# microsoft/tutel

Measured on NVIDIA H100. Metric: moe_layer_fwd_bwd_tokens_per_sec, higher is better.
Workload: dtype bf16; 1 GPU; model=helloworld moe_layer top-2 8-expert ffn(relu) model_dim=4096 hidden=14336, global_batch=16, seq_len=512, parallelism=ep1 (8 local experts/GPU), a2a_ffn_overlap_degree=1, cuda_graph=True, launches_per_graph_replay=15

## Files before the change

### csrc/gemm_sm90.cu

```cuda
#include "gemm_sm90.h"

#include <cuda.h>
#include <cuda_bf16.h>
#include <cuda_fp16.h>

#include <cstdio>
#include <cstdlib>
#include <mutex>

#include "ptx.cuh"

namespace tb {

struct GemmArgs {
  int M, N, K, G;
  int b_group_div;
  int tiles_m, tiles_n;
  long long num_tiles;

  void* d;
  long long ldd, d_group_stride;
  const unsigned long long* d_ptr_table;
  int out_dtype;

// ... 17 lines not shown
  long long colsum_group_stride;
  const float* scale_a;
  long long scale_a_group_stride;
  const float* scale_b;
  long long scale_b_group_stride;

  const uint32_t* wait_flags;
  int wait_rows_per_flag, wait_flags_per_group;
  uint32_t wait_target;
  const unsigned long long* signal_ptr_table;
  int group_rot, group_mod;
};

namespace {

constexpr int kThreads = 384;
constexpr int kSwizzleBytes = 128;
constexpr int kSmemLimit = 232448;

template <int BN_>
struct Cfg {
  static constexpr int BM = 128;
  static constexpr int BN = BN_;
  static constexpr bool WIDE = BN_ == 256;
  static constexpr int A_BYTES = BM * kSwizzleBytes;
  static constexpr int B_BYTES = BN * kSwizzleBytes;
  static constexpr int STAGE_BYTES = A_BYTES + B_BYTES;
  static constexpr int EPI_COLS = 128;
  static constexpr int EPI_PITCH = EPI_COLS + 8;
  static constexpr int EPI_WARP_BYTES = 16 * EPI_PITCH * 4;
  static constexpr int EPI_BYTES = WIDE ? 0 : 8 * EPI_WARP_BYTES;
  static constexpr int OUT_BOX_BYTES = BM * kSwizzleBytes;
  static constexpr int OUT_TILE_BYTES = WIDE ? BM * BN * 2 : 0;
  static constexpr int COLSUM_BYTES = WIDE ? 2 * BN * 4 : 0;
  static constexpr int BAR_BYTES = 512;
  static constexpr int STAGES = WIDE ? 3 : 4;
  static constexpr int MAXNREG = WIDE ? 168 : 144;
  static constexpr int CONSUMER_REGS = WIDE ? 232 : 192;
  static constexpr int SMEM_BYTES = STAGES * STAGE_BYTES + 1024 + OUT_TILE_BYTES + BAR_BYTES + EPI_BYTES + COLSUM_BYTES;
  static_assert((STAGES * STAGE_BYTES) % 1024 == 0, "the output tile must stay 1024B aligned for the 128B swizzle");
  static_assert(WIDE || SMEM_BYTES + 2 * 1024 <= 228 * 1024, "no room for the push kernel");
  static_assert(SMEM_BYTES <= kSmemLimit, "");
  static_assert(128 * 40 + 256 * CONSUMER_REGS <= 65536 && 384 * MAXNREG <= 65536, "register budget");
};

struct TileCoord {
  int g, m_blk, n_blk;
};

template <int kBand>
__device__ __forceinline__ TileCoord decode_tile(long long t, int tiles_m, int tiles_n) {
  const int per_group = tiles_m * tiles_n;
  TileCoord c;
  c.g = static_cast<int>(t / per_group);
  int r = static_cast<int>(t - static_cast<long long>(c.g) * per_group);
  const int band_tiles = kBand * tiles_n;
  const int band = r / band_tiles;
  const int first_m = band * kBand;
  const int rows_in_band = min(kBand, tiles_m - first_m);
  r -= band * band_tiles;
  c.m_blk = first_m + r % rows_in_band;
  c.n_blk = r / rows_in_band;
  return c;
}

__device__ __forceinline__ int rotate_group(int g, int rot, int mod) {
  if (mod > 1) {
    const int base = (g / mod) * mod;
    return base + (g - base + rot) % mod;
  }
  if (mod < -1) {
    const int m = -mod;
// ... 88 lines not shown
    else a = g[j] * fast_sigmoid(g[j]);
    o[j] = a * u[j];
  }
}
template <int ACT>
__device__ __forceinline__ void glu_bwd_seg(const float* r, const float* g, float* u, float* o) {
#pragma unroll
  for (int j = 0; j < 32; ++j) {
    const float dh = r[j];
    float a, da;
    if constexpr (ACT == ACT_RELU) {
      a = fmaxf(g[j], 0.0f);
      da = g[j] > 0.0f ? 1.0f : 0.0f;
    } else if constexpr (ACT == ACT_GELU) {
      const float cdf = 0.5f * (1.0f + erff(g[j] * 0.70710678118654752f));
      a = g[j] * cdf;
      da = cdf + g[j] * 0.3989422804014327f * __expf(-0.5f * g[j] * g[j]);
    } else {
      const float sg = fast_sigmoid(g[j]);
      a = g[j] * sg;
      da = sg * (1.0f + g[j] * (1.0f - sg));
    }
    o[j] = dh * u[j] * da;
    u[j] = dh * a;
  }
}

enum WideMain : int { WM_NONE, WM_BIAS, WM_RELU_BWD, WM_ADD, WM_GELU_BWD, WM_SILU_BWD };

__device__ __forceinline__ uint32_t out_tile_off(int j, int swz) {
  return static_cast<uint32_t>((j >> 3) * (128 * kSwizzleBytes) + (((j & 7) ^ swz) << 4));
}

__device__ __forceinline__ void wide_scale(float (&acc)[128], float sa0, float sa1, const float* sb, int n_lane, int N) {
#pragma unroll
  for (int j = 0; j < 32; ++j) {
    const int n = n_lane + 8 * j;
    if (sb != nullptr && n < N) {
      const float2 s = *reinterpret_cast<const float2*>(sb + n);
      acc[4 * j] *= sa0 * s.x; acc[4 * j + 1] *= sa0 * s.y;
      acc[4 * j + 2] *= sa1 * s.x; acc[4 * j + 3] *= sa1 * s.y;
    } else {
      acc[4 * j] *= sa0; acc[4 * j + 1] *= sa0;
      acc[4 * j + 2] *= sa1; acc[4 * j + 3] *= sa1;
    }
  }
}

template <int WM>
__device__ __forceinline__ void wide_main(float (&acc)[128], const uint8_t* row0, int swz, const uint8_t* bias_g,
                                          bool bias_f32, bool bias_bf16, int n_lane, int N, bool out_bf16, float alpha) {
#pragma unroll
  for (int j = 0; j < 32; ++j) {
    if constexpr (WM == WM_NONE) {
#pragma unroll
      for (int c = 0; c < 4; ++c) acc[4 * j + c] *= alpha;
    } else if constexpr (WM == WM_BIAS) {
      const int n = n_lane + 8 * j;
      float2 b = make_float2(0.0f, 0.0f);
      if (n < N)
        b = bias_f32 ? *reinterpret_cast<const float2*>(bias_g + n * 4)
                     : unpack2(*reinterpret_cast<const uint32_t*>(bias_g + n * 2), bias_bf16);
      acc[4 * j] += b.x; acc[4 * j + 1] += b.y;
      acc[4 * j + 2] += b.x; acc[4 * j + 3] += b.y;
    } else {
      const uint32_t o = out_tile_off(j, swz);
#pragma unroll
      for (int h = 0; h < 2; ++h) {
        const float2 f = unpack2(*reinterpret_cast<const uint32_t*>(row0 + h * 8 * kSwizzleBytes + o), out_bf16);
        float& v0 = acc[4 * j + 2 * h];
        float& v1 = acc[4 * j + 2 * h + 1];
        if constexpr (WM == WM_RELU_BWD) { v0 = relu_bwd(v0, f.x); v1 = relu_bwd(v1, f.y); }
        else if constexpr (WM == WM_ADD) { v0 += f.x; v1 += f.y; }
        else if constexpr (WM == WM_GELU_BWD) { v0 = gelu_bwd(v0, f.x); v1 = gelu_bwd(v1, f.y); }
        else { v0 = silu_bwd(v0, f.x); v1 = silu_bwd(v1, f.y); }
      }
    }
  }
}

template <int ACT>
__device__ __forceinline__ void wide_act(float (&acc)[128]) {
#pragma unroll
  for (int i = 0; i < 128; ++i) {
    if constexpr (ACT == ACT_RELU) acc[i] = fmaxf(acc[i], 0.0f);
    else if constexpr (ACT == ACT_GELU) acc[i] = gelu_erf(acc[i]);
    else acc[i] = silu(acc[i]);
  }
}

__device__ __forceinline__ void wide_stage(const float (&acc)[128], uint8_t* row0, int swz, bool out_bf16) {
#pragma unroll
  for (int j = 0; j < 32; ++j) {
    const uint32_t o = out_tile_off(j, swz);
    *reinterpret_cast<uint32_t*>(row0 + o) = pack2(acc[4 * j], acc[4 * j + 1], out_bf16);
    *reinterpret_cast<uint32_t*>(row0 + 8 * kSwizzleBytes + o) = pack2(acc[4 * j + 2], acc[4 * j + 3], out_bf16);
  }
}

__device__ __forceinline__ void wide_colsum(const float (&acc)[128], bool ok0, bool ok1, int lane, float* colrow) {
  float s[64];
#pragma unroll
  for (int j = 0; j < 32; ++j) {
#pragma unroll
    for (int c = 0; c < 2; ++c) s[2 * j + c] = (ok0 ? acc[4 * j + c] : 0.0f) + (ok1 ? acc[4 * j + 2 + c] : 0.0f);
  }
#pragma unroll
  for (int off = 16; off >= 4; off >>= 1) {
    const bool upper = (lane & off) != 0;
#pragma unroll
    for (int i = 0; i < 2 * off; ++i) {
      const float send = upper ? s[i] : s[i + 2 * off];
      const float recv = __shfl_xor_sync(0xffffffffu, send, off);
      s[i] = (upper ? s[i + 2 * off] : s[i]) + recv;
    }
  }
  float* base = colrow + 32 * (lane >> 2) + 2 * (lane & 3);
#pragma unroll
  for (int i = 0; i < 8; ++i) atomicAdd(base + 8 * (i >> 1) + (i & 1), s[i]);
}

struct OutTileStore {
  const uint8_t* tile;
  uint32_t tile_smem;
  int m0, n0, m_valid, N, g;
  long long group_stride, ld;
  bool straddle;
  int ct;
  bool writer;
};
__device__ __forceinline__ void flush_out_tile(const OutTileStore& s, const CUtensorMap* map, uint8_t* dst, bool wait_read) {
  constexpr int kChunks = 256 / 8;
  ptx::fence_proxy_async_smem();
  ptx::named_bar_sync(1, 256);
  if (s.straddle) {
    for (int i = s.ct; i < 128 * kChunks; i += 256) {
      const int r = i / kChunks, ch = i % kChunks;
      const int m = s.m0 + r, n = s.n0 + ch * 8;
      if (m < s.m_valid && n < s.N) {
        const uint4 v = *reinterpret_cast<const uint4*>(s.tile + (ch >> 3) * (128 * kSwizzleBytes) + r * kSwizzleBytes +
                                                        (((ch & 7) ^ (r & 7)) << 4));
        *reinterpret_cast<uint4*>(dst + (static_cast<long long>(s.g) * s.group_stride + static_cast<long long>(m) * s.ld + n) * 2) = v;
      }
    }
    ptx::named_bar_sync(1, 256);
    return;
  }
  if (s.writer) {
    for (int b = 0; b < 4; ++b)
      if (s.n0 + 64 * b < s.N) ptx::tma_store_3d(map, s.tile_smem + b * (128 * kSwizzleBytes), s.n0 + 64 * b, s.m0, s.g);
    ptx::bulk_commit_group();
    if (wait_read) ptx::bulk_wait_group_read<0>();
  }
  if (wait_read) ptx::named_bar_sync(1, 256);
}

template <int BN_, bool A_MN, bool B_MN, int DT>
__global__ void __maxnreg__(Cfg<BN_>::MAXNREG)
gemm_sm90_kernel(const __grid_constant__ CUtensorMap tmA, const __grid_constant__ CUtensorMap tmB,
                 const __grid_constant__ CUtensorMap tmB2, const __grid_constant__ CUtensorMap tmD,
                 const __grid_constant__ CUtensorMap tmAux, const __grid_constant__ CUtensorMap tmD2,
                 const GemmArgs args) {
  using C = Cfg<BN_>;
  constexpr int BN = C::BN;
  extern __shared__ uint8_t smem_raw[];

  const int warp = __shfl_sync(0xffffffffu, static_cast<int>(threadIdx.x >> 5), 0);
  const int lane = threadIdx.x & 31;

  const uint32_t smem_base = (ptx::smem_u32(smem_raw) + 1023u) & ~1023u;
  constexpr int stages = C::STAGES;
  const uint32_t out_base = smem_base + static_cast<uint32_t>(stages) * C::STAGE_BYTES;
  const uint32_t bar_base = out_base + C::OUT_TILE_BYTES;
  auto smem_a = [&](int s) { return smem_base + s * C::STAGE_BYTES; };
  auto smem_b = [&](int s) { return smem_base + s * C::STAGE_BYTES + C::A_BYTES; };
  auto full_bar = [&](int s) { return bar_base + 8u * s; };
  auto empty_bar = [&](int s) { return bar_base + 64u + 8u * s; };
  const uint32_t aux_full = bar_base + 128u;
  const uint32_t out_empty = bar_base + 136u;
  const uint32_t epi_base = bar_base + C::BAR_BYTES;
  float* epi_ptr = reinterpret_cast<float*>(smem_raw + (epi_base - ptx::smem_u32(smem_raw)));
  uint8_t* out_tile = smem_raw + (out_base - ptx::smem_u32(smem_raw));
  float* colsum_rows = epi_ptr;
  const bool aux_tma = C::WIDE && (args.epilogue == EPI_RELU_BWD || args.epilogue == EPI_ADD || args.epilogue == EPI_ACT_BWD);

  if (warp == 0 && ptx::elect_one()) {
    ptx::prefetch_tensormap(&tmA);
    ptx::prefetch_tensormap(&tmB);
    if (args.dual) ptx::prefetch_tensormap(&tmB2);
    if (C::WIDE) ptx::prefetch_tensormap(&tmD);
    if (aux_tma) ptx::prefetch_tensormap(&tmAux);
  }
  if (warp == 1 && lane == 0) {
    for (int s = 0; s < stages; ++s) {
      ptx::mbar_init(full_bar(s), 1);
      ptx::mbar_init(empty_bar(s), 2);
    }
    ptx::mbar_init(aux_full, 1);
    ptx::mbar_init(out_empty, 1);
    ptx::fence_mbar_init();
  }
  if constexpr (C::WIDE) {
    for (int i = threadIdx.x; i < 2 * BN; i += kThreads) colsum_rows[i] = 0.0f;
  }
  __syncthreads();

  constexpr int kEltBytes = (DT == DT_E4M3 || DT == DT_E5M2) ? 1 : 2;
  static_assert(kEltBytes == 2 || (!A_MN && !B_MN), "8-bit operands are K-major only");
  const int num_kb = (args.K * kEltBytes + kSwizzleBytes - 1) / kSwizzleBytes;
  constexpr int bk_elems = kSwizzleBytes / kEltBytes;
  const long long tile_step = gridDim.x;
  const long long tile_first = blockIdx.x;
  constexpr int kBand = 16;
  const bool dual = !C::WIDE && args.dual != 0;
  const int tile_n = dual ? BN / 2 : BN;
  const int kb_out_free = min(2, num_kb - 1);

  if (warp < 4) {
    ptx::setmaxnreg_dec<40>();
    if (warp == 0) {
      int s = 0;
      uint32_t ph = 0;
      uint32_t it = 0;
      int seen_group = -1;
      unsigned long long seen_mask = 0ull;
      for (long long t = tile_first; t < args.num_tiles; t += tile_step) {
        TileCoord tc = decode_tile<kBand>(t, args.tiles_m, args.tiles_n);
        tc.g = rotate_group(tc.g, args.group_rot, args.group_mod);
        if (args.row_counts != nullptr && tc.m_blk * C::BM >= args.row_counts[tc.g]) continue;
        const int m0 = tc.m_blk * C::BM;
        const int n0 = tc.n_blk * BN;
        const int gb = tc.g / args.b_group_div;
        if (args.wait_flags != nullptr) {
          if (tc.g != seen_group) { seen_group = tc.g; seen_mask = 0ull; }
          const int f0 = (tc.m_blk * C::BM) / args.wait_rows_per_flag;
          const int f1 = (min(tc.m_blk * C::BM + C::BM, args.M) - 1) / args.wait_rows_per_flag;
          unsigned long long need = 0ull;
          for (int f = f0; f <= f1; ++f) need |= 1ull << (f & 63);
          if ((seen_mask & need) != need) {
            if (lane == 0) {
              for (int f = f0; f <= f1; ++f)
                if (!((seen_mask >> (f & 63)) & 1ull))
                  ptx::wait_flag_ge_sys_quiet(args.wait_flags + static_cast<long long>(tc.g) * args.wait_flags_per_group + f,
                                        args.wait_target);
              ptx::fence_proxy_async_global();
            }
            __syncwarp();
            seen_mask |= need;
          }
        }
        for (int kb = 0; kb < num_kb; ++kb) {
          ptx::mbar_wait_quiet(empty_bar(s), ph ^ 1u);
          if (ptx::elect_one()) {
            const uint32_t fb = full_bar(s);
            ptx::mbar_expect_tx(fb, C::STAGE_BYTES);
            const int k0 = kb * bk_elems;
            constexpr int chunk_elems = kSwizzleBytes / kEltBytes;
            constexpr int chunk_bytes = bk_elems * kSwizzleBytes;
            if constexpr (!A_MN) {
              ptx::tma_load_3d(smem_a(s), &tmA, fb, k0, m0, tc.g);
            } else {
              for (int c = 0; c < C::BM / chunk_elems; ++c)
                ptx::tma_load_3d(smem_a(s) + c * chunk_bytes, &tmA, fb, m0 + c * chunk_elems, k0, tc.g);
            }
            if (!dual) {
              if constexpr (!B_MN) {
                ptx::tma_load_3d(smem_b(s), &tmB, fb, k0, n0, gb);
              } else {
                for (int c = 0; c < BN / chunk_elems; ++c)
                  ptx::tma_load_3d(smem_b(s) + c * chunk_bytes, &tmB, fb, n0 + c * chunk_elems, k0, gb);
              }
            } else {
              const int nb0 = tc.n_blk * (BN / 2);
              if constexpr (!B_MN) {
                ptx::tma_load_3d(smem_b(s), &tmB, fb, k0, nb0, gb);
                ptx::tma_load_3d(smem_b(s) + (BN / 2) * kSwizzleBytes, &tmB2, fb, k0, nb0, gb);
              } else {
                constexpr int half_chunks = (BN / 2) / chunk_elems;
                for (int c = 0; c < 2 * half_chunks; ++c)
                  ptx::tma_load_3d(smem_b(s) + c * chunk_bytes, c < half_chunks ? &tmB : &tmB2, fb,
                                   nb0 + (c % half_chunks) * chunk_elems, k0, gb);
              }
            }
          }
          __syncwarp();
          if (++s == stages) { s = 0; ph ^= 1u; }
          if (aux_tma && kb == kb_out_free) {
            ptx::mbar_wait_quiet(out_empty, (it & 1u) ^ 1u);
            if (ptx::elect_one()) {
              ptx::mbar_expect_tx(aux_full, C::OUT_TILE_BYTES);
              for (int b = 0; b < BN / 64; ++b)
                ptx::tma_load_3d(out_base + b * C::OUT_BOX_BYTES, &tmAux, aux_full, n0 + 64 * b, m0, tc.g);
            }
            __syncwarp();
          }
        }
        ++it;
      }
    }
  } else {
    ptx::setmaxnreg_inc<C::CONSUMER_REGS>();
    const int cw = warp - 4;
    const int wg = cw >> 2;
    const bool wg_leader = (threadIdx.x & 127) == 0;
    int s = 0;
    uint32_t ph = 0;
    constexpr uint32_t kMnChunkBytes = 64u * kSwizzleBytes;
    constexpr uint32_t kMnKStep = 16u * kSwizzleBytes;
    constexpr uint32_t a_lbo = A_MN ? kMnChunkBytes : 16u;
    constexpr uint32_t b_lbo = B_MN ? kMnChunkBytes : 16u;
    constexpr uint32_t a_kstep = (A_MN ? kMnKStep : 32u) >> 4;
    constexpr uint32_t b_kstep = (B_MN ? kMnKStep : 32u) >> 4;
    constexpr uint32_t desc_hi = (1024u >> 4) | (1u << 30);
    const uint32_t a_lo0 = (((smem_a(0) + static_cast<uint32_t>(wg) * 8192u) >> 4) & 0x3FFFu) | ((a_lbo >> 4) << 16);
    const uint32_t b_lo0 = ((smem_b(0) >> 4) & 0x3FFFu) | ((b_lbo >> 4) << 16);

    const bool out16 = (args.out_dtype != DT_FP32);
    const bool out_bf16 = (args.out_dtype == DT_BF16);
    const bool glu = !C::WIDE && (args.epilogue == EPI_GLU || args.epilogue == EPI_GLU_BWD);
    float* epi_warp = epi_ptr + cw * 16 * C::EPI_PITCH;
    const float* epi_row = epi_warp + (lane & 15) * C::EPI_PITCH;
    const int col_half = (lane >> 4) * 32;
    auto load_acc = [&](int col, float* v) {
#pragma unroll
      for (int q = 0; q < 8; ++q) {
        const float4 t4 = *reinterpret_cast<const float4*>(epi_row + col + q * 4);
        v[q * 4] = t4.x; v[q * 4 + 1] = t4.y; v[q * 4 + 2] = t4.z; v[q * 4 + 3] = t4.w;
      }
    };
    const int ct = threadIdx.x - 128;
    const bool out_writer = ct == 0;
    const int r0 = cw * 16 + (lane >> 2);
    const int swz = lane >> 2;
    uint8_t* row0 = out_tile + r0 * kSwizzleBytes + (lane & 3) * 4;
    const int wmain = args.epilogue == EPI_NONE ? WM_NONE
                    : args.epilogue == EPI_ADD ? WM_ADD
                    : args.epilogue == EPI_RELU_BWD ? WM_RELU_BWD
                    : args.epilogue == EPI_ACT_BWD ? (args.act == ACT_GELU ? WM_GELU_BWD : args.act == ACT_SILU ? WM_SILU_BWD : WM_RELU_BWD)
                    : WM_BIAS;
    uint32_t it = 0;

    for (long long t = tile_first; t < args.num_tiles; t += tile_step) {
      TileCoord tc = decode_tile<kBand>(t, args.tiles_m, args.tiles_n);
      tc.g = rotate_group(tc.g, args.group_rot, args.group_mod);
      int m_valid = args.M;
      if (args.row_counts != nullptr) {
        m_valid = min(args.M, args.row_counts[tc.g]);
        if (tc.m_blk * C::BM >= m_valid) continue;
      }
      float acc[BN / 2];
      if constexpr (C::WIDE) {
#pragma unroll
        for (int i = 0; i < BN / 2; ++i) acc[i] = 0.0f;
      }
      int prev_s = 0;
      for (int kb = 0; kb < num_kb; ++kb) {
        ptx::mbar_wait_quiet(full_bar(s), ph);
        const uint32_t a_lo = a_lo0 + static_cast<uint32_t>(s) * (C::STAGE_BYTES >> 4);
        const uint32_t b_lo = b_lo0 + static_cast<uint32_t>(s) * (C::STAGE_BYTES >> 4);
        ptx::wgmma_fence();
#pragma unroll
        for (int k = 0; k < 4; ++k) {
          const uint64_t ad = (static_cast<uint64_t>(desc_hi) << 32) | (a_lo + k * a_kstep);
          const uint64_t bd = (static_cast<uint64_t>(desc_hi) << 32) | (b_lo + k * b_kstep);
          if constexpr (BN == 256) ptx::wgmma_m64n256<DT, A_MN, B_MN>(acc, ad, bd, (kb | k) != 0);
          else ptx::wgmma_m64n128<DT, A_MN, B_MN>(acc, ad, bd, (kb | k) != 0);
        }
        ptx::wgmma_commit();
        if constexpr (C::WIDE) {
          if (out_writer && it > 0 && kb == kb_out_free) {
            ptx::bulk_wait_group_read<0>();
            ptx::mbar_arrive(out_empty);
          }
          __syncwarp();
        }
        if (kb > 0) {
          ptx::wgmma_wait<1>();
          if (wg_leader) ptx::mbar_arrive(empty_bar(prev_s));
        }
        prev_s = s;
        if (++s == stages) { s = 0; ph ^= 1u; }
      }
      ptx::wgmma_wait<0>();
      if (wg_leader) ptx::mbar_arrive(empty_bar(prev_s));

      if constexpr (C::WIDE) {
        const int m0 = tc.m_blk * C::BM, n0 = tc.n_blk * BN;
        const int gb = tc.g / args.b_group_div;
        const bool ok0 = m0 + r0 < m_valid, ok1 = m0 + r0 + 8 < m_valid;
        const int n_lane = n0 + 2 * (lane & 3);
        const bool straddle = m0 + C::BM > m_valid && m_valid < args.M;
        if (args.scale_a != nullptr || args.scale_b != nullptr) {
          const float* sa = args.scale_a != nullptr ? args.scale_a + static_cast<long long>(tc.g) * args.scale_a_group_stride + m0 + r0 : nullptr;
          const float sa0 = (sa != nullptr && ok0) ? sa[0] : 1.0f;
          const float sa1 = (sa != nullptr && ok1) ? sa[8] : 1.0f;
          const float* sb = args.scale_b != nullptr ? args.scale_b + static_cast<long long>(gb) * args.scale_b_group_stride : nullptr;
          wide_scale(acc, sa0, sa1, sb, n_lane, args.N);
        }
        const uint8_t* bias_g = nullptr;
        if (args.bias != nullptr)
          bias_g = reinterpret_cast<const uint8_t*>(args.bias) +
                   static_cast<long long>(gb) * args.bias_group_stride * (args.bias_is_fp32 ? 4 : 2);
        const uint32_t out_free_parity = (it & 1u) ^ 1u;

        const OutTileStore st{out_tile, out_base, m0, n0, m_valid, args.N, tc.g, args.d_group_stride, args.ldd, straddle, ct,
                              out_writer};

        if (wmain == WM_BIAS) {
          if (bias_g != nullptr)
            wide_main<WM_BIAS>(acc, row0, swz, bias_g, args.bias_is_fp32 != 0, args.bias_is_bf16 != 0, n_lane, args.N, out_bf16, 1.0f);
          if (args.d2 != nullptr && (args.epilogue == EPI_BIAS_GELU || args.epilogue == EPI_BIAS_SILU)) {
            ptx::mbar_wait_quiet(out_empty, out_free_parity);
            wide_stage(acc, row0, swz, out_bf16);
            flush_out_tile(st, &tmD2, reinterpret_cast<uint8_t*>(args.d2), true);
          }
          if (args.epilogue == EPI_BIAS_RELU) wide_act<ACT_RELU>(acc);
          else if (args.epilogue == EPI_BIAS_GELU) wide_act<ACT_GELU>(acc);
          else if (args.epilogue == EPI_BIAS_SILU) wide_act<ACT_SILU>(acc);
        } else if (wmain == WM_NONE) {
          if (args.alpha != 1.0f) wide_main<WM_NONE>(acc, row0, swz, nullptr, false, false, n_lane, args.N, out_bf16, args.alpha);
        } else {
          ptx::mbar_wait_quiet(aux_full, it & 1u);
          if (wmain == WM_RELU_BWD) wide_main<WM_RELU_BWD>(acc, row0, swz, nullptr, false, false, n_lane, args.N, out_bf16, 1.0f);
          else if (wmain == WM_ADD) wide_main<WM_ADD>(acc, row0, swz, nullptr, false, false, n_lane, args.N, out_bf16, 1.0f);
          else if (wmain == WM_GELU_BWD) wide_main<WM_GELU_BWD>(acc, row0, swz, nullptr, false, false, n_lane, args.N, out_bf16, 1.0f);
          else wide_main<WM_SILU_BWD>(acc, row0, swz, nullptr, false, false, n_lane, args.N, out_bf16, 1.0f);
        }
        if (!aux_tma) ptx::mbar_wait_quiet(out_empty, out_free_parity);
        wide_stage(acc, row0, swz, out_bf16);
        float* colrow = colsum_rows + (it & 1u) * BN;
        if (args.colsum != nullptr) wide_colsum(acc, ok0, ok1, lane, colrow);
        flush_out_tile(st, &tmD, reinterpret_cast<uint8_t*>(args.d), false);
        if (args.colsum != nullptr && ct < BN / 4) {
          float4* src = reinterpret_cast<float4*>(colrow) + ct;
          const float4 v = *src;
          *src = make_float4(0.0f, 0.0f, 0.0f, 0.0f);
          const int n = n0 + 4 * ct;
          if (n < args.N) {
            float* cs = args.colsum + static_cast<long long>(gb) * args.colsum_group_stride + n;
            if ((reinterpret_cast<uintptr_t>(cs) & 15) == 0) {
              ptx::red_add_v4_f32(cs, v.x, v.y, v.z, v.w);
            } else {
              atomicAdd(cs, v.x); atomicAdd(cs + 1, v.y); atomicAdd(cs + 2, v.z); atomicAdd(cs + 3, v.w);
            }
          }
        }
        ++it;
        continue;
      }

      {
        const int fr = lane >> 2, fc = (lane & 3) * 2;
#pragma unroll
        for (int j = 0; j < C::EPI_COLS / 8; ++j) {
          *reinterpret_cast<float2*>(epi_warp + fr * C::EPI_PITCH + j * 8 + fc) = make_float2(acc[4 * j], acc[4 * j + 1]);
          *reinterpret_cast<float2*>(epi_warp + (fr + 8) * C::EPI_PITCH + j * 8 + fc) = make_float2(acc[4 * j + 2], acc[4 * j + 3]);
        }
      }
      __syncwarp();

      const int m = tc.m_blk * C::BM + cw * 16 + (lane & 15);
      const bool row_ok = m < m_valid;
      const int gb = tc.g / args.b_group_div;
      uint8_t* d_base = (args.d_ptr_table != nullptr)
                            ? reinterpret_cast<uint8_t*>(args.d_ptr_table[tc.g])
                            : reinterpret_cast<uint8_t*>(args.d) +
                                  static_cast<long long>(tc.g) * args.d_group_stride * (out16 ? 2 : 4);
      uint8_t* d_row = d_base + static_cast<long long>(m) * args.ldd * (out16 ? 2 : 4);
      const uint8_t* aux_row = nullptr;
      if (args.aux != nullptr)
        aux_row = reinterpret_cast<const uint8_t*>(args.aux) +
                  (static_cast<long long>(tc.g) * args.aux_group_stride + static_cast<long long>(m) * args.ld_aux) * 2;
      const uint8_t* aux2_row = nullptr;
      if (args.aux2 != nullptr)
        aux2_row = reinterpret_cast<const uint8_t*>(args.aux2) +
                   (static_cast<long long>(tc.g) * args.aux_group_stride + static_cast<long long>(m) * args.ld_aux) * 2;
      const uint8_t* bias_g = nullptr;
      if (args.bias != nullptr)
        bias_g = reinterpret_cast<const uint8_t*>(args.bias) +
// ... 157 lines not shown
        if (args.colsum != nullptr) {
          float s[32];
#pragma unroll
          for (int j = 0; j < 32; ++j) s[j] = row_ok ? v[j] : 0.0f;
#pragma unroll
          for (int off = 8; off >= 1; off >>= 1) {
            const bool upper = (lane & off) != 0;
#pragma unroll
            for (int i = 0; i < 2 * off; ++i) {
              const float send = upper ? s[i] : s[i + 2 * off];
              const float recv = __shfl_xor_sync(0xffffffffu, send, off);
              s[i] = (upper ? s[i + 2 * off] : s[i]) + recv;
            }
          }
          const int cc = 2 * (lane & 15);
          float* cs = args.colsum + static_cast<long long>(gb) * args.colsum_group_stride + n + cc;
          if (cc < ncols) {
            atomicAdd(cs, s[0]);
            atomicAdd(cs + 1, s[1]);
          }
        }
        store_seg(d_row, n, ncols, v);
      }
      }
      __syncwarp();
      if (args.signal_ptr_table != nullptr) {
        asm volatile("bar.sync 1, 256;" ::: "memory");
        if (cw == 0 && lane == 0) {
          ptx::fence_acq_rel_sys();
          ptx::red_add_release_sys(reinterpret_cast<uint32_t*>(args.signal_ptr_table[tc.g]), 1u);
        }
      }
    }
    if constexpr (C::WIDE) {
      if (out_writer) ptx::bulk_wait_group<0>();
    }
  }
}

using EncodeTiledFn = CUresult (*)(CUtensorMap*, CUtensorMapDataType, cuuint32_t, void*, const cuuint64_t*,
                                   const cuuint64_t*, const cuuint32_t*, const cuuint32_t*, CUtensorMapInterleave,
                                   CUtensorMapSwizzle, CUtensorMapL2promotion, CUtensorMapFloatOOBfill);

EncodeTiledFn get_encode_fn() {
  static EncodeTiledFn fn = nullptr;
  static std::once_flag once;
  std::call_once(once, [] {
    void* p = nullptr;
    cudaDriverEntryPointQueryResult q;
    if (cudaGetDriverEntryPoint("cuTensorMapEncodeTiled", &p, cudaEnableDefault, &q) == cudaSuccess &&
        q == cudaDriverEntryPointSuccess)
      fn = reinterpret_cast<EncodeTiledFn>(p);
  });
  return fn;
}

bool make_operand_map(CUtensorMap* map, const void* base, int dtype, bool mn_major, long long rows_mn,
                      long long k, long long ld, long long group_stride, int groups, int box_mn_kmajor,
                      const char** why) {
  EncodeTiledFn enc = get_encode_fn();
  if (enc == nullptr) { *why = "cuTensorMapEncodeTiled unavailable"; return false; }
  const int eb = (dtype == DT_E4M3 || dtype == DT_E5M2) ? 1 : 2;
  CUtensorMapDataType dt = eb == 1 ? CU_TENSOR_MAP_DATA_TYPE_UINT8
                                   : (dtype == DT_BF16 ? CU_TENSOR_MAP_DATA_TYPE_BFLOAT16 : CU_TENSOR_MAP_DATA_TYPE_FLOAT16);
  if ((reinterpret_cast<uintptr_t>(base) & 15) || ((ld * eb) & 15) || ((group_stride * eb) & 15)) {
    *why = "operand base/stride must be 16-byte aligned";
    return false;
  }
  cuuint64_t dims[3];
// ... 77 lines not shown
  int sms = sm_count_cache[dev & 63];
  if (p.max_ctas > 0) sms = p.max_ctas < sms ? p.max_ctas : sms;

  const bool dual = p.epilogue == EPI_GLU;
  if (dual && (p.b2 == nullptr || p.out_dtype == DT_FP32)) { *why = "EPI_GLU needs b2 and a 16-bit output"; return cudaErrorInvalidValue; }
  if (p.epilogue == EPI_GLU_BWD && (p.aux == nullptr || p.aux2 == nullptr || p.d2 == nullptr || p.out_dtype == DT_FP32)) {
    *why = "EPI_GLU_BWD needs aux, aux2, d2 and a 16-bit output";
    return cudaErrorInvalidValue;
  }
  if ((p.epilogue == EPI_GLU || p.epilogue == EPI_GLU_BWD) && p.d_ptr_table != nullptr) { *why = "GLU epilogues write local outputs only"; return cudaErrorInvalidValue; }
  const bool uses_aux = p.epilogue == EPI_RELU_BWD || p.epilogue == EPI_ADD || p.epilogue == EPI_GLU_BWD || p.epilogue == EPI_ACT_BWD;
  if (uses_aux && (p.aux == nullptr || p.out_dtype == DT_FP32 ||
                   ((reinterpret_cast<uintptr_t>(p.aux) | reinterpret_cast<uintptr_t>(p.aux2)) & 15) || ((p.ld_aux * 2) & 15) ||
                   ((p.aux_group_stride * 2) & 15))) {
    *why = "this epilogue needs a 16-byte aligned 16-bit aux operand";
    return cudaErrorInvalidValue;
  }
  const int groups_b = (p.G + (p.b_group_div > 0 ? p.b_group_div : 1) - 1) / (p.b_group_div > 0 ? p.b_group_div : 1);
  if ((p.G > 1 && (p.a_group_stride == 0 || (p.d_ptr_table == nullptr && p.d_group_stride == 0) ||
                   (uses_aux && p.aux_group_stride == 0))) ||
      (groups_b > 1 && p.b_group_stride == 0)) {
    *why = "group strides of A, B, aux and the output must be nonzero when there is more than one group";
    return cudaErrorInvalidValue;
  }
  const int mod_abs = p.group_mod < 0 ? -p.group_mod : p.group_mod;
  if (mod_abs > 1 && (p.G % mod_abs != 0 || p.group_rot < 0)) {
    *why = "G must be a multiple of |group_mod|, and group_rot must not be negative";
    return cudaErrorInvalidValue;
  }
  if (p.alpha != 1.0f && p.epilogue != EPI_NONE) { *why = "alpha is applied by EPI_NONE only"; return cudaErrorInvalidValue; }
  if (p.cta_group < 0 || p.cta_group > 2) { *why = "cta_group must be 0, 1 or 2"; return cudaErrorInvalidValue; }
  if (p.block_n != 0 && p.block_n != 128 && p.block_n != 256) { *why = "block_n must be 0, 128 or 256"; return cudaErrorInvalidValue; }

  const bool wide = p.block_n != 128 && p.wait_flags == nullptr && p.signal_ptr_table == nullptr && p.d_ptr_table == nullptr &&
                    p.epilogue != EPI_GLU && p.epilogue != EPI_GLU_BWD && p.out_dtype != DT_FP32;
  constexpr int bm = 128;
  const int bn = wide ? 256 : 128;
  GemmArgs a{};
  a.M = p.M; a.N = p.N; a.K = p.K; a.G = p.G;
  a.b_group_div = p.b_group_div > 0 ? p.b_group_div : 1;
  a.tiles_m = (p.M + bm - 1) / bm;
  a.tiles_n = dual ? (p.N + bn / 2 - 1) / (bn / 2) : (p.N + bn - 1) / bn;
  a.num_tiles = static_cast<long long>(a.tiles_m) * a.tiles_n * p.G;
  a.d = p.d; a.ldd = p.ldd; a.d_group_stride = p.d_group_stride; a.d_ptr_table = p.d_ptr_table;
  a.out_dtype = p.out_dtype;
  a.epilogue = p.epilogue; a.alpha = p.alpha;
  a.bias = p.bias; a.bias_group_stride = p.bias_group_stride; a.bias_is_fp32 = 0;
  a.bias_is_bf16 = (eb == 2) ? (p.in_dtype == DT_BF16) : (p.out_dtype == DT_BF16);
  a.aux = p.aux; a.ld_aux = p.ld_aux; a.aux_group_stride = p.aux_group_stride;
  a.aux2 = p.aux2; a.d2 = p.d2; a.d3 = p.d3; a.dual = dual ? 1 : 0; a.act = p.act; a.scale_b2 = p.scale_b2;
  a.row_counts = p.row_counts;
  a.colsum = p.colsum; a.colsum_group_stride = p.colsum_group_stride;
  a.scale_a = p.scale_a; a.scale_a_group_stride = p.scale_a_group_stride;
  a.scale_b = p.scale_b; a.scale_b_group_stride = p.scale_b_group_stride;
  a.wait_flags = p.wait_flags; a.wait_rows_per_flag = p.wait_rows_per_flag > 0 ? p.wait_rows_per_flag : bm;
  a.wait_flags_per_group = p.wait_flags_per_group; a.wait_target = p.wait_target;
  a.signal_ptr_table = p.signal_ptr_table;
  a.group_rot = p.group_rot; a.group_mod = p.group_mod;

  CUtensorMap ta, tb_;
  const int gB = (p.G + a.b_group_div - 1) / a.b_group_div;
  if (!make_operand_map(&ta, p.a, p.in_dtype, p.a_mn_major, p.M, p.K, p.lda, p.a_group_stride, p.G, bm, why))
    return cudaErrorInvalidValue;
  const int b_box = dual ? bn / 2 : bn;
  if (!make_operand_map(&tb_, p.b, p.in_dtype, p.b_mn_major, p.N, p.K, p.ldb, p.b_group_stride, gB, b_box, why))
    return cudaErrorInvalidValue;
  CUtensorMap tb2 = tb_;
  if (dual && !make_operand_map(&tb2, p.b2, p.in_dtype, p.b_mn_major, p.N, p.K, p.ldb, p.b_group_stride, gB, b_box, why))
// ... 45 lines not shown
```

### csrc/ptx.cuh

```cuda
#pragma once
#include <cstdint>
#include <cstdio>
#include <cuda.h>
#include <cuda_runtime.h>

#ifndef TB_SPIN_TIMEOUT_NS
#define TB_SPIN_TIMEOUT_NS 300000000000ull
#endif

static __constant__ unsigned long long tb_spin_timeout_ns = TB_SPIN_TIMEOUT_NS;

namespace ptx {

__device__ __forceinline__ uint32_t smem_u32(const void* p) {
  return static_cast<uint32_t>(__cvta_generic_to_shared(p));
}

__device__ __forceinline__ uint64_t globaltimer_ns() {
  uint64_t t;
  asm volatile("mov.u64 %0, %%globaltimer;" : "=l"(t));
  return t;
}

__device__ __forceinline__ uint32_t elect_one() {
// ... 136 lines not shown
    if (globaltimer_ns() - t0 > tb_spin_timeout_ns) __trap();
  }
}

__device__ __forceinline__ uint4 ld_nc_v4(const void* p) {
  uint4 r;
  asm volatile("ld.global.nc.L1::no_allocate.v4.u32 {%0,%1,%2,%3}, [%4];"
               : "=r"(r.x), "=r"(r.y), "=r"(r.z), "=r"(r.w)
               : "l"(p));
  return r;
}
__device__ __forceinline__ uint4 ld_v4(const void* p) {
  uint4 r;
  asm volatile("ld.global.v4.u32 {%0,%1,%2,%3}, [%4];" : "=r"(r.x), "=r"(r.y), "=r"(r.z), "=r"(r.w) : "l"(p));
  return r;
}
__device__ __forceinline__ void st_na_v4(void* p, const uint4& v) {
  asm volatile("st.global.L1::no_allocate.v4.u32 [%0], {%1,%2,%3,%4};" ::"l"(p), "r"(v.x), "r"(v.y), "r"(v.z),
               "r"(v.w)
               : "memory");
}

__device__ __forceinline__ void prefetch_tensormap(const void* tmap) {
  asm volatile("prefetch.tensormap [%0];" ::"l"(tmap) : "memory");
}

__device__ __forceinline__ void tma_load_3d(uint32_t smem_dst, const void* tmap, uint32_t bar, int c0, int c1,
                                            int c2) {
  asm volatile(
      "cp.async.bulk.tensor.3d.shared::cluster.global.mbarrier::complete_tx::bytes"
      " [%0], [%1, {%3, %4, %5}], [%2];" ::"r"(smem_dst),
      "l"(tmap), "r"(bar), "r"(c0), "r"(c1), "r"(c2)
      : "memory");
}
__device__ __forceinline__ void prefetch_l2_bulk(const void* gptr, uint32_t bytes) {
  asm volatile("cp.async.bulk.prefetch.L2.global [%0], %1;" ::"l"(gptr), "r"(bytes) : "memory");
}

__device__ __forceinline__ void tma_store_3d(const void* tmap, uint32_t smem_src, int c0, int c1, int c2) {
  asm volatile("cp.async.bulk.tensor.3d.global.shared::cta.bulk_group [%0, {%2, %3, %4}], [%1];" ::"l"(tmap),
               "r"(smem_src), "r"(c0), "r"(c1), "r"(c2)
               : "memory");
}
__device__ __forceinline__ void bulk_commit_group() { asm volatile("cp.async.bulk.commit_group;" ::: "memory"); }
template <int N>
__device__ __forceinline__ void bulk_wait_group_read() { asm volatile("cp.async.bulk.wait_group.read %0;" ::"n"(N) : "memory"); }
template <int N>
__device__ __forceinline__ void bulk_wait_group() { asm volatile("cp.async.bulk.wait_group %0;" ::"n"(N) : "memory"); }

__device__ __forceinline__ void named_bar_sync(int id, int count) {
  asm volatile("bar.sync %0, %1;" ::"r"(id), "r"(count) : "memory");
}

__device__ __forceinline__ void red_add_v4_f32(float* p, float a, float b, float c, float d) {
  asm volatile("red.global.add.v4.f32 [%0], {%1, %2, %3, %4};" ::"l"(p), "f"(a), "f"(b), "f"(c), "f"(d) : "memory");
}

__device__ __forceinline__ void wgmma_fence() { asm volatile("wgmma.fence.sync.aligned;" ::: "memory"); }
__device__ __forceinline__ void wgmma_commit() { asm volatile("wgmma.commit_group.sync.aligned;" ::: "memory"); }
template <int N>
__device__ __forceinline__ void wgmma_wait() { asm volatile("wgmma.wait_group.sync.aligned %0;" ::"n"(N) : "memory"); }

enum WgmmaType : int { WG_BF16 = 0, WG_FP16 = 1, WG_E4M3 = 3, WG_E5M2 = 4 };

#define TB_ACC8(d, o) "+f"(d[o]), "+f"(d[o + 1]), "+f"(d[o + 2]), "+f"(d[o + 3]), "+f"(d[o + 4]), "+f"(d[o + 5]), "+f"(d[o + 6]), "+f"(d[o + 7])
#define TB_ACC64(d) TB_ACC8(d, 0), TB_ACC8(d, 8), TB_ACC8(d, 16), TB_ACC8(d, 24), TB_ACC8(d, 32), TB_ACC8(d, 40), TB_ACC8(d, 48), TB_ACC8(d, 56)
// ... 67 lines not shown
```

Before: 441,300 tokens/s.

## Move wide-tile epilogue stores, colsum reduction and side loads to dedicated producer warp

Adds a dedicated warp (warp 1) that owns the output-tile drain for the wide 128x256 GEMM path. It issues the TMA stores, reduces per-warp column-sum partials and does the global atomics, and prefetches the next aux tile. Per-tile bias and scale_b vectors are bulk-copied into double-buffered shared memory, so consumers read them from smem instead of global. Consumer warpgroups now only stage the tile and arrive on an mbarrier, which removes the named-barrier flush and the colsum smem atomics from the math critical path. In exchange it uses more shared memory, and the wide path now requires 16-byte-aligned bias/scale pointers, so misaligned inputs fall back to the narrow path.

```diff
diff --git a/csrc/gemm_sm90.cu b/csrc/gemm_sm90.cu
--- a/csrc/gemm_sm90.cu
+++ b/csrc/gemm_sm90.cu
@@ -73,12 +73,16 @@
   static constexpr int EPI_BYTES = WIDE ? 0 : 8 * EPI_WARP_BYTES;
   static constexpr int OUT_BOX_BYTES = BM * kSwizzleBytes;
   static constexpr int OUT_TILE_BYTES = WIDE ? BM * BN * 2 : 0;
-  static constexpr int COLSUM_BYTES = WIDE ? 2 * BN * 4 : 0;
+  static constexpr int COLSUM_BYTES = WIDE ? 8 * BN * 4 : 0;
+  static constexpr int SIDE_BIAS_BYTES = BN * 4;
+  static constexpr int SIDE_SLOT_BYTES = SIDE_BIAS_BYTES + BN * 4;
+  static constexpr int SIDE_BYTES = WIDE ? 2 * SIDE_SLOT_BYTES : 0;
   static constexpr int BAR_BYTES = 512;
   static constexpr int STAGES = WIDE ? 3 : 4;
   static constexpr int MAXNREG = WIDE ? 168 : 144;
   static constexpr int CONSUMER_REGS = WIDE ? 232 : 192;
-  static constexpr int SMEM_BYTES = STAGES * STAGE_BYTES + 1024 + OUT_TILE_BYTES + BAR_BYTES + EPI_BYTES + COLSUM_BYTES;
+  static constexpr int SMEM_BYTES =
+      STAGES * STAGE_BYTES + 1024 + OUT_TILE_BYTES + BAR_BYTES + EPI_BYTES + COLSUM_BYTES + SIDE_BYTES;
   static_assert((STAGES * STAGE_BYTES) % 1024 == 0, "the output tile must stay 1024B aligned for the 128B swizzle");
   static_assert(WIDE || SMEM_BYTES + 2 * 1024 <= 228 * 1024, "no room for the push kernel");
   static_assert(SMEM_BYTES <= kSmemLimit, "");
@@ -233,11 +237,11 @@
   return static_cast<uint32_t>((j >> 3) * (128 * kSwizzleBytes) + (((j & 7) ^ swz) << 4));
 }
 
-__device__ __forceinline__ void wide_scale(float (&acc)[128], float sa0, float sa1, const float* sb, int n_lane, int N) {
+__device__ __forceinline__ void wide_scale(float (&acc)[128], float sa0, float sa1, const float* sb, int n_lane, int n_lim) {
 #pragma unroll
   for (int j = 0; j < 32; ++j) {
     const int n = n_lane + 8 * j;
-    if (sb != nullptr && n < N) {
+    if (sb != nullptr && n < n_lim) {
       const float2 s = *reinterpret_cast<const float2*>(sb + n);
       acc[4 * j] *= sa0 * s.x; acc[4 * j + 1] *= sa0 * s.y;
       acc[4 * j + 2] *= sa1 * s.x; acc[4 * j + 3] *= sa1 * s.y;
@@ -249,8 +253,8 @@
 }
 
 template <int WM>
-__device__ __forceinline__ void wide_main(float (&acc)[128], const uint8_t* row0, int swz, const uint8_t* bias_g,
-                                          bool bias_f32, bool bias_bf16, int n_lane, int N, bool out_bf16, float alpha) {
+__device__ __forceinline__ void wide_main(float (&acc)[128], const uint8_t* row0, int swz, const uint8_t* bias_s,
+                                          bool bias_f32, bool bias_bf16, int n_lane, int n_lim, bool out_bf16, float alpha) {
 #pragma unroll
   for (int j = 0; j < 32; ++j) {
     if constexpr (WM == WM_NONE) {
@@ -259,9 +263,9 @@
     } else if constexpr (WM == WM_BIAS) {
       const int n = n_lane + 8 * j;
       float2 b = make_float2(0.0f, 0.0f);
-      if (n < N)
-        b = bias_f32 ? *reinterpret_cast<const float2*>(bias_g + n * 4)
-                     : unpack2(*reinterpret_cast<const uint32_t*>(bias_g + n * 2), bias_bf16);
+      if (n < n_lim)
+        b = bias_f32 ? *reinterpret_cast<const float2*>(bias_s + n * 4)
+                     : unpack2(*reinterpret_cast<const uint32_t*>(bias_s + n * 2), bias_bf16);
       acc[4 * j] += b.x; acc[4 * j + 1] += b.y;
       acc[4 * j + 2] += b.x; acc[4 * j + 3] += b.y;
     } else {
@@ -299,6 +303,16 @@
   }
 }
 
+template <int OFF>
+__device__ __forceinline__ void colsum_halve(float (&s)[64], int lane) {
+  const bool upper = (lane & OFF) != 0;
+#pragma unroll
+  for (int i = 0; i < 2 * OFF; ++i) {
+    const float lo = s[i], hi = s[i + 2 * OFF];
+    const float recv = __shfl_xor_sync(0xffffffffu, upper ? lo : hi, OFF);
+    s[i] = (upper ? hi : lo) + recv;
+  }
+}
 __device__ __forceinline__ void wide_colsum(const float (&acc)[128], bool ok0, bool ok1, int lane, float* colrow) {
   float s[64];
 #pragma unroll
@@ -306,54 +320,33 @@
 #pragma unroll
     for (int c = 0; c < 2; ++c) s[2 * j + c] = (ok0 ? acc[4 * j + c] : 0.0f) + (ok1 ? acc[4 * j + 2 + c] : 0.0f);
   }
-#pragma unroll
-  for (int off = 16; off >= 4; off >>= 1) {
-    const bool upper = (lane & off) != 0;
-#pragma unroll
-    for (int i = 0; i < 2 * off; ++i) {
-      const float send = upper ? s[i] : s[i + 2 * off];
-      const float recv = __shfl_xor_sync(0xffffffffu, send, off);
-      s[i] = (upper ? s[i + 2 * off] : s[i]) + recv;
-    }
-  }
+  colsum_halve<16>(s, lane);
+  colsum_halve<8>(s, lane);
+  colsum_halve<4>(s, lane);
   float* base = colrow + 32 * (lane >> 2) + 2 * (lane & 3);
 #pragma unroll
-  for (int i = 0; i < 8; ++i) atomicAdd(base + 8 * (i >> 1) + (i & 1), s[i]);
-}
-
-struct OutTileStore {
-  const uint8_t* tile;
-  uint32_t tile_smem;
-  int m0, n0, m_valid, N, g;
-  long long group_stride, ld;
-  bool straddle;
-  int ct;
-  bool writer;
-};
-__device__ __forceinline__ void flush_out_tile(const OutTileStore& s, const CUtensorMap* map, uint8_t* dst, bool wait_read) {
+  for (int q = 0; q < 4; ++q) *reinterpret_cast<float2*>(base + 8 * q) = make_float2(s[2 * q], s[2 * q + 1]);
+}
+
+__device__ __forceinline__ void hand_over_tile(const uint8_t* tile, bool straddle, int m0, int n0, int m_valid, int N, int g,
+                                               long long group_stride, long long ld, uint8_t* dst, int ct, int lane,
+                                               uint32_t out_full) {
   constexpr int kChunks = 256 / 8;
   ptx::fence_proxy_async_smem();
-  ptx::named_bar_sync(1, 256);
-  if (s.straddle) {
-    for (int i = s.ct; i < 128 * kChunks; i += 256) {
+  if (straddle) {
+    ptx::named_bar_sync(1, 256);
+    for (int i = ct; i < 128 * kChunks; i += 256) {
       const int r = i / kChunks, ch = i % kChunks;
-      const int m = s.m0 + r, n = s.n0 + ch * 8;
-      if (m < s.m_valid && n < s.N) {
-        const uint4 v = *reinterpret_cast<const uint4*>(s.tile + (ch >> 3) * (128 * kSwizzleBytes) + r * kSwizzleBytes +
+      const int m = m0 + r, n = n0 + ch * 8;
+      if (m < m_valid && n < N) {
+        const uint4 v = *reinterpret_cast<const uint4*>(tile + (ch >> 3) * (128 * kSwizzleBytes) + r * kSwizzleBytes +
                                                         (((ch & 7) ^ (r & 7)) << 4));
-        *reinterpret_cast<uint4*>(dst + (static_cast<long long>(s.g) * s.group_stride + static_cast<long long>(m) * s.ld + n) * 2) = v;
+        *reinterpret_cast<uint4*>(dst + (static_cast<long long>(g) * group_stride + static_cast<long long>(m) * ld + n) * 2) = v;
       }
     }
-    ptx::named_bar_sync(1, 256);
-    return;
-  }
-  if (s.writer) {
-    for (int b = 0; b < 4; ++b)
-      if (s.n0 + 64 * b < s.N) ptx::tma_store_3d(map, s.tile_smem + b * (128 * kSwizzleBytes), s.n0 + 64 * b, s.m0, s.g);
-    ptx::bulk_commit_group();
-    if (wait_read) ptx::bulk_wait_group_read<0>();
-  }
-  if (wait_read) ptx::named_bar_sync(1, 256);
+  }
+  __syncwarp();
+  if (lane == 0) ptx::mbar_arrive(out_full);
 }
 
 template <int BN_, bool A_MN, bool B_MN, int DT>
@@ -379,11 +372,17 @@
   auto empty_bar = [&](int s) { return bar_base + 64u + 8u * s; };
   const uint32_t aux_full = bar_base + 128u;
   const uint32_t out_empty = bar_base + 136u;
+  const uint32_t out_full = bar_base + 144u;
+  auto side_full = [&](uint32_t slot) { return bar_base + 152u + 8u * slot; };
   const uint32_t epi_base = bar_base + C::BAR_BYTES;
   float* epi_ptr = reinterpret_cast<float*>(smem_raw + (epi_base - ptx::smem_u32(smem_raw)));
   uint8_t* out_tile = smem_raw + (out_base - ptx::smem_u32(smem_raw));
-  float* colsum_rows = epi_ptr;
+  float* colsum_part = epi_ptr;
+  const uint32_t side_base = epi_base + C::COLSUM_BYTES;
   const bool aux_tma = C::WIDE && (args.epilogue == EPI_RELU_BWD || args.epilogue == EPI_ADD || args.epilogue == EPI_ACT_BWD);
+  const bool side_bias = C::WIDE && args.bias != nullptr && !aux_tma && args.epilogue != EPI_NONE;
+  const bool side_in = side_bias || (C::WIDE && args.scale_b != nullptr);
+  const bool pre_act = C::WIDE && args.d2 != nullptr && (args.epilogue == EPI_BIAS_GELU || args.epilogue == EPI_BIAS_SILU);
 
   if (warp == 0 && ptx::elect_one()) {
     ptx::prefetch_tensormap(&tmA);
@@ -391,6 +390,7 @@
     if (args.dual) ptx::prefetch_tensormap(&tmB2);
     if (C::WIDE) ptx::prefetch_tensormap(&tmD);
     if (aux_tma) ptx::prefetch_tensormap(&tmAux);
+    if (pre_act) ptx::prefetch_tensormap(&tmD2);
   }
   if (warp == 1 && lane == 0) {
     for (int s = 0; s < stages; ++s) {
@@ -399,10 +399,10 @@
     }
     ptx::mbar_init(aux_full, 1);
     ptx::mbar_init(out_empty, 1);
+    ptx::mbar_init(out_full, 8);
+    ptx::mbar_init(side_full(0), 1);
+    ptx::mbar_init(side_full(1), 1);
     ptx::fence_mbar_init();
-  }
-  if constexpr (C::WIDE) {
-    for (int i = threadIdx.x; i < 2 * BN; i += kThreads) colsum_rows[i] = 0.0f;
   }
   __syncthreads();
 
@@ -415,14 +415,12 @@
   constexpr int kBand = 16;
   const bool dual = !C::WIDE && args.dual != 0;
   const int tile_n = dual ? BN / 2 : BN;
-  const int kb_out_free = min(2, num_kb - 1);
 
   if (warp < 4) {
     ptx::setmaxnreg_dec<40>();
     if (warp == 0) {
       int s = 0;
       uint32_t ph = 0;
-      uint32_t it = 0;
       int seen_group = -1;
       unsigned long long seen_mask = 0ull;
       for (long long t = tile_first; t < args.num_tiles; t += tile_step) {
@@ -486,18 +484,101 @@
           }
           __syncwarp();
           if (++s == stages) { s = 0; ph ^= 1u; }
-          if (aux_tma && kb == kb_out_free) {
-            ptx::mbar_wait_quiet(out_empty, (it & 1u) ^ 1u);
-            if (ptx::elect_one()) {
-              ptx::mbar_expect_tx(aux_full, C::OUT_TILE_BYTES);
-              for (int b = 0; b < BN / 64; ++b)
-                ptx::tma_load_3d(out_base + b * C::OUT_BOX_BYTES, &tmAux, aux_full, n0 + 64 * b, m0, tc.g);
+        }
+      }
+    } else if (C::WIDE && warp == 1) {
+      const int side_es = args.bias_is_fp32 ? 4 : 2;
+      uint32_t it = 0;
+      uint32_t outs = 0;
+      TileCoord prev{};
+      int prev_m_valid = 0;
+      auto drain = [&](const CUtensorMap* map, const TileCoord& tc, int m_valid, bool colsum, bool has_next, TileCoord next) {
+        const int m0 = tc.m_blk * C::BM, n0 = tc.n_blk * BN;
+        const bool straddle = m0 + C::BM > m_valid && m_valid < args.M;
+        ptx::mbar_wait_quiet(out_full, outs & 1u);
+        if (!straddle && lane == 0) {
+          for (int b = 0; b < BN / 64; ++b)
+            if (n0 + 64 * b < args.N) ptx::tma_store_3d(map, out_base + b * C::OUT_BOX_BYTES, n0 + 64 * b, m0, tc.g);
+          ptx::bulk_commit_group();
+        }
+        if (colsum) {
+#pragma unroll 1
+          for (int h = 0; h < 2; ++h) {
+            const int c = 128 * h + 4 * lane;
+            float4 v = *reinterpret_cast<const float4*>(colsum_part + c);
+#pragma unroll
+            for (int w = 1; w < 8; ++w) {
+              const float4 p = *reinterpret_cast<const float4*>(colsum_part + w * BN + c);
+              v.x += p.x; v.y += p.y; v.z += p.z; v.w += p.w;
             }
-            __syncwarp();
-          }
-        }
+            const int n = n0 + c;
+            if (n < args.N) {
+              float* cs = args.colsum + static_cast<long long>(tc.g / args.b_group_div) * args.colsum_group_stride + n;
+              if ((reinterpret_cast<uintptr_t>(cs) & 15) == 0) {
+                ptx::red_add_v4_f32(cs, v.x, v.y, v.z, v.w);
+              } else {
+                atomicAdd(cs, v.x); atomicAdd(cs + 1, v.y); atomicAdd(cs + 2, v.z); atomicAdd(cs + 3, v.w);
+              }
+            }
+          }
+        }
+        __syncwarp();
+        if (lane == 0) {
+          ptx::bulk_wait_group_read<0>();
+          if (has_next) {
+            ptx::mbar_expect_tx(aux_full, C::OUT_TILE_BYTES);
+            for (int b = 0; b < BN / 64; ++b)
+              ptx::tma_load_3d(out_base + b * C::OUT_BOX_BYTES, &tmAux, aux_full, next.n_blk * BN + 64 * b,
+                               next.m_blk * C::BM, next.g);
+          } else if (!aux_tma) {
+            ptx::mbar_arrive(out_empty);
+          }
+        }
+        __syncwarp();
+        ++outs;
+      };
+      for (long long t = tile_first; t < args.num_tiles; t += tile_step) {
+        TileCoord tc = decode_tile<kBand>(t, args.tiles_m, args.tiles_n);
+        tc.g = rotate_group(tc.g, args.group_rot, args.group_mod);
+        int m_valid = args.M;
+        if (args.row_counts != nullptr) {
+          m_valid = min(args.M, args.row_counts[tc.g]);
+          if (tc.m_blk * C::BM >= m_valid) continue;
+        }
+        if (it > 0 && pre_act) drain(&tmD2, prev, prev_m_valid, false, false, prev);
+        if (side_in) {
+          if (it > 0 && !pre_act) ptx::mbar_wait_quiet(out_full, outs & 1u);
+          const int n0 = tc.n_blk * BN;
+          const int gb = tc.g / args.b_group_div;
+          const int cols = min(BN, args.N - n0);
+          const uint32_t slot = side_base + (it & 1u) * C::SIDE_SLOT_BYTES;
+          const uint8_t* bsrc = reinterpret_cast<const uint8_t*>(args.bias) +
+                                (static_cast<long long>(gb) * args.bias_group_stride + n0) * side_es;
+          const float* ssrc = args.scale_b + static_cast<long long>(gb) * args.scale_b_group_stride + n0;
+          if (lane == 0) {
+            const uint32_t bar = side_full(it & 1u);
+            ptx::mbar_expect_tx(bar, (side_bias ? cols * side_es : 0) + (args.scale_b != nullptr ? cols * 4 : 0));
+            if (side_bias) ptx::bulk_load(slot, bsrc, cols * side_es, bar);
+            if (args.scale_b != nullptr) ptx::bulk_load(slot + C::SIDE_BIAS_BYTES, ssrc, cols * 4, bar);
+          }
+          __syncwarp();
+        }
+        if (it > 0) drain(&tmD, prev, prev_m_valid, args.colsum != nullptr, aux_tma, tc);
+        else if (aux_tma && lane == 0) {
+          ptx::mbar_expect_tx(aux_full, C::OUT_TILE_BYTES);
+          for (int b = 0; b < BN / 64; ++b)
+            ptx::tma_load_3d(out_base + b * C::OUT_BOX_BYTES, &tmAux, aux_full, tc.n_blk * BN + 64 * b, tc.m_blk * C::BM, tc.g);
+        }
+        __syncwarp();
+        prev = tc;
+        prev_m_valid = m_valid;
         ++it;
       }
+      if (it > 0) {
+        if (pre_act) drain(&tmD2, prev, prev_m_valid, false, false, prev);
+        drain(&tmD, prev, prev_m_valid, args.colsum != nullptr, false, prev);
+      }
+      if (lane == 0) ptx::bulk_wait_group<0>();
     }
   } else {
     ptx::setmaxnreg_inc<C::CONSUMER_REGS>();
@@ -530,7 +611,6 @@
       }
     };
     const int ct = threadIdx.x - 128;
-    const bool out_writer = ct == 0;
     const int r0 = cw * 16 + (lane >> 2);
     const int swz = lane >> 2;
     uint8_t* row0 = out_tile + r0 * kSwizzleBytes + (lane & 3) * 4;
@@ -540,6 +620,7 @@
                     : args.epilogue == EPI_ACT_BWD ? (args.act == ACT_GELU ? WM_GELU_BWD : args.act == ACT_SILU ? WM_SILU_BWD : WM_RELU_BWD)
                     : WM_BIAS;
     uint32_t it = 0;
+    uint32_t outs = 0;
 
     for (long long t = tile_first; t < args.num_tiles; t += tile_step) {
       TileCoord tc = decode_tile<kBand>(t, args.tiles_m, args.tiles_n);
@@ -568,13 +649,6 @@
           else ptx::wgmma_m64n128<DT, A_MN, B_MN>(acc, ad, bd, (kb | k) != 0);
         }
         ptx::wgmma_commit();
-        if constexpr (C::WIDE) {
-          if (out_writer && it > 0 && kb == kb_out_free) {
-            ptx::bulk_wait_group_read<0>();
-            ptx::mbar_arrive(out_empty);
-          }
-          __syncwarp();
-        }
         if (kb > 0) {
           ptx::wgmma_wait<1>();
           if (wg_leader) ptx::mbar_arrive(empty_bar(prev_s));
@@ -587,65 +661,49 @@
 
       if constexpr (C::WIDE) {
         const int m0 = tc.m_blk * C::BM, n0 = tc.n_blk * BN;
-        const int gb = tc.g / args.b_group_div;
         const bool ok0 = m0 + r0 < m_valid, ok1 = m0 + r0 + 8 < m_valid;
-        const int n_lane = n0 + 2 * (lane & 3);
+        const int n_lane = 2 * (lane & 3);
+        const int n_lim = args.N - n0;
         const bool straddle = m0 + C::BM > m_valid && m_valid < args.M;
+        const uint8_t* side = reinterpret_cast<const uint8_t*>(colsum_part + 8 * BN) + (it & 1u) * C::SIDE_SLOT_BYTES;
+        if (side_in) ptx::mbar_wait_quiet(side_full(it & 1u), (it >> 1) & 1u);
         if (args.scale_a != nullptr || args.scale_b != nullptr) {
           const float* sa = args.scale_a != nullptr ? args.scale_a + static_cast<long long>(tc.g) * args.scale_a_group_stride + m0 + r0 : nullptr;
           const float sa0 = (sa != nullptr && ok0) ? sa[0] : 1.0f;
           const float sa1 = (sa != nullptr && ok1) ? sa[8] : 1.0f;
-          const float* sb = args.scale_b != nullptr ? args.scale_b + static_cast<long long>(gb) * args.scale_b_group_stride : nullptr;
-          wide_scale(acc, sa0, sa1, sb, n_lane, args.N);
-        }
-        const uint8_t* bias_g = nullptr;
-        if (args.bias != nullptr)
-          bias_g = reinterpret_cast<const uint8_t*>(args.bias) +
-                   static_cast<long long>(gb) * args.bias_group_stride * (args.bias_is_fp32 ? 4 : 2);
-        const uint32_t out_free_parity = (it & 1u) ^ 1u;
-
-        const OutTileStore st{out_tile, out_base, m0, n0, m_valid, args.N, tc.g, args.d_group_stride, args.ldd, straddle, ct,
-                              out_writer};
+          const float* sb = args.scale_b != nullptr ? reinterpret_cast<const float*>(side + C::SIDE_BIAS_BYTES) : nullptr;
+          wide_scale(acc, sa0, sa1, sb, n_lane, n_lim);
+        }
+        auto wait_out_free = [&]() { ptx::mbar_wait_quiet(out_empty, (outs & 1u) ^ 1u); };
+        auto hand_over = [&](uint8_t* dst) {
+          hand_over_tile(out_tile, straddle, m0, n0, m_valid, args.N, tc.g, args.d_group_stride, args.ldd, dst, ct, lane, out_full);
+          ++outs;
+        };
 
         if (wmain == WM_BIAS) {
-          if (bias_g != nullptr)
-            wide_main<WM_BIAS>(acc, row0, swz, bias_g, args.bias_is_fp32 != 0, args.bias_is_bf16 != 0, n_lane, args.N, out_bf16, 1.0f);
-          if (args.d2 != nullptr && (args.epilogue == EPI_BIAS_GELU || args.epilogue == EPI_BIAS_SILU)) {
-            ptx::mbar_wait_quiet(out_empty, out_free_parity);
+          if (side_bias)
+            wide_main<WM_BIAS>(acc, row0, swz, side, args.bias_is_fp32 != 0, args.bias_is_bf16 != 0, n_lane, n_lim, out_bf16, 1.0f);
+          if (pre_act) {
+            wait_out_free();
             wide_stage(acc, row0, swz, out_bf16);
-            flush_out_tile(st, &tmD2, reinterpret_cast<uint8_t*>(args.d2), true);
+            hand_over(reinterpret_cast<uint8_t*>(args.d2));
           }
           if (args.epilogue == EPI_BIAS_RELU) wide_act<ACT_RELU>(acc);
           else if (args.epilogue == EPI_BIAS_GELU) wide_act<ACT_GELU>(acc);
           else if (args.epilogue == EPI_BIAS_SILU) wide_act<ACT_SILU>(acc);
         } else if (wmain == WM_NONE) {
-          if (args.alpha != 1.0f) wide_main<WM_NONE>(acc, row0, swz, nullptr, false, false, n_lane, args.N, out_bf16, args.alpha);
+          if (args.alpha != 1.0f) wide_main<WM_NONE>(acc, row0, swz, nullptr, false, false, n_lane, n_lim, out_bf16, args.alpha);
         } else {
           ptx::mbar_wait_quiet(aux_full, it & 1u);
-          if (wmain == WM_RELU_BWD) wide_main<WM_RELU_BWD>(acc, row0, swz, nullptr, false, false, n_lane, args.N, out_bf16, 1.0f);
-          else if (wmain == WM_ADD) wide_main<WM_ADD>(acc, row0, swz, nullptr, false, false, n_lane, args.N, out_bf16, 1.0f);
-          else if (wmain == WM_GELU_BWD) wide_main<WM_GELU_BWD>(acc, row0, swz, nullptr, false, false, n_lane, args.N, out_bf16, 1.0f);
-          else wide_main<WM_SILU_BWD>(acc, row0, swz, nullptr, false, false, n_lane, args.N, out_bf16, 1.0f);
-        }
-        if (!aux_tma) ptx::mbar_wait_quiet(out_empty, out_free_parity);
+          if (wmain == WM_RELU_BWD) wide_main<WM_RELU_BWD>(acc, row0, swz, nullptr, false, false, n_lane, n_lim, out_bf16, 1.0f);
+          else if (wmain == WM_ADD) wide_main<WM_ADD>(acc, row0, swz, nullptr, false, false, n_lane, n_lim, out_bf16, 1.0f);
+          else if (wmain == WM_GELU_BWD) wide_main<WM_GELU_BWD>(acc, row0, swz, nullptr, false, false, n_lane, n_lim, out_bf16, 1.0f);
+          else wide_main<WM_SILU_BWD>(acc, row0, swz, nullptr, false, false, n_lane, n_lim, out_bf16, 1.0f);
+        }
+        if (!aux_tma) wait_out_free();
         wide_stage(acc, row0, swz, out_bf16);
-        float* colrow = colsum_rows + (it & 1u) * BN;
-        if (args.colsum != nullptr) wide_colsum(acc, ok0, ok1, lane, colrow);
-        flush_out_tile(st, &tmD, reinterpret_cast<uint8_t*>(args.d), false);
-        if (args.colsum != nullptr && ct < BN / 4) {
-          float4* src = reinterpret_cast<float4*>(colrow) + ct;
-          const float4 v = *src;
-          *src = make_float4(0.0f, 0.0f, 0.0f, 0.0f);
-          const int n = n0 + 4 * ct;
-          if (n < args.N) {
-            float* cs = args.colsum + static_cast<long long>(gb) * args.colsum_group_stride + n;
-            if ((reinterpret_cast<uintptr_t>(cs) & 15) == 0) {
-              ptx::red_add_v4_f32(cs, v.x, v.y, v.z, v.w);
-            } else {
-              atomicAdd(cs, v.x); atomicAdd(cs + 1, v.y); atomicAdd(cs + 2, v.z); atomicAdd(cs + 3, v.w);
-            }
-          }
-        }
+        if (args.colsum != nullptr) wide_colsum(acc, ok0, ok1, lane, colsum_part + cw * BN);
+        hand_over(reinterpret_cast<uint8_t*>(args.d));
         ++it;
         continue;
       }
@@ -869,9 +927,6 @@
         }
       }
     }
-    if constexpr (C::WIDE) {
-      if (out_writer) ptx::bulk_wait_group<0>();
-    }
   }
 }
 
@@ -1015,8 +1070,11 @@
   if (p.cta_group < 0 || p.cta_group > 2) { *why = "cta_group must be 0, 1 or 2"; return cudaErrorInvalidValue; }
   if (p.block_n != 0 && p.block_n != 128 && p.block_n != 256) { *why = "block_n must be 0, 128 or 256"; return cudaErrorInvalidValue; }
 
+  const bool side_aligned =
+      ((reinterpret_cast<uintptr_t>(p.bias) | static_cast<uintptr_t>(p.bias_group_stride * 2)) & 15) == 0 &&
+      ((reinterpret_cast<uintptr_t>(p.scale_b) | static_cast<uintptr_t>(p.scale_b_group_stride * 4)) & 15) == 0;
   const bool wide = p.block_n != 128 && p.wait_flags == nullptr && p.signal_ptr_table == nullptr && p.d_ptr_table == nullptr &&
-                    p.epilogue != EPI_GLU && p.epilogue != EPI_GLU_BWD && p.out_dtype != DT_FP32;
+                    p.epilogue != EPI_GLU && p.epilogue != EPI_GLU_BWD && p.out_dtype != DT_FP32 && side_aligned;
   constexpr int bm = 128;
   const int bn = wide ? 256 : 128;
   GemmArgs a{};
diff --git a/csrc/ptx.cuh b/csrc/ptx.cuh
--- a/csrc/ptx.cuh
+++ b/csrc/ptx.cuh
@@ -192,6 +192,11 @@
       " [%0], [%1, {%3, %4, %5}], [%2];" ::"r"(smem_dst),
       "l"(tmap), "r"(bar), "r"(c0), "r"(c1), "r"(c2)
       : "memory");
+}
+__device__ __forceinline__ void bulk_load(uint32_t smem_dst, const void* gsrc, uint32_t bytes, uint32_t bar) {
+  asm volatile("cp.async.bulk.shared::cluster.global.mbarrier::complete_tx::bytes [%0], [%1], %2, [%3];" ::"r"(smem_dst),
+               "l"(gsrc), "r"(bytes), "r"(bar)
+               : "memory");
 }
 __device__ __forceinline__ void prefetch_l2_bulk(const void* gptr, uint32_t bytes) {
   asm volatile("cp.async.bulk.prefetch.L2.global [%0], %1;" ::"l"(gptr), "r"(bytes) : "memory");
```

After: 459,400 tokens/s (median of 6 runs). 1.04x the previous value.
